# qucontrol/krotov

Hardware: AMD Instinct MI355X
Metric: state*timestep propagations/s (Krotov iterations/s in iterations_per_sec), 256-objective N=64 ensemble (higher is better)
Workload: dtype f64

## Files before the change

### include/krotov_hip.h

```cpp
#ifndef KROTOV_HIP_H
#define KROTOV_HIP_H

#include <stddef.h>
#include <stdint.h>

#ifdef __cplusplus
extern "C" {
#endif

typedef struct kh_engine kh_engine;

typedef struct kh_cdouble {
    double re, im;
} kh_cdouble;

enum kh_status {
    KH_OK = 0,
    KH_ERR_INVALID = -1,
    KH_ERR_HIP = -2,
    KH_ERR_UNSUPPORTED = -3,
    KH_ERR_TIMEOUT = -4,
    KH_ERR_NOMEM = -5
};

// ... 125 lines not shown

int kh_expect(kh_engine *engine, const kh_cdouble *states_dev, const kh_cdouble *const *e_ops, int32_t n_e,
              kh_cdouble *out_dev, void *stream);

int kh_chi_boundary(kh_engine *engine, const kh_cdouble *targets_dev,
                    const kh_cdouble *psi_T_dev, const kh_cdouble *c_dev,
                    const kh_cdouble *d_dev, kh_cdouble *chi_T_dev,
                    double *chi_norms_dev, void *stream);

int kh_check(kh_engine *engine);

int kh_last_stats(kh_engine *engine, double stats[4]);

int kh_series_tables(int32_t real_spectrum, double tol, double *theta , double *ratios );

int kh_series_tables_defect(double tol, double theta_cap, double defect, double *theta ,
                            double *ratios );

int kh_series_tables_odd(double tol, double *theta , double *c0 , double *rows );

int32_t kh_ell_rows_of(int32_t N);
int kh_ell_layout(int32_t N, int32_t n_ops, const kh_csr *ops_host, int32_t *E, int32_t *Ec, int32_t *off,
                  kh_cdouble *vals, int32_t E_cap);
int kh_ell_layout_global(int32_t N, int32_t n_ops, const kh_csr *ops_host, int32_t *E, int32_t *Ec, int32_t *off,
                         kh_cdouble *vals, int32_t E_cap);

int kh_set_row_split(kh_engine *engine, int workgroups_per_objective);
int kh_ellsplit_rows(int32_t N, int32_t S, int32_t part, int32_t *first, int32_t *count);

int kh_debug_occupy(kh_engine *engine, int32_t workgroups, double milliseconds, void *stream);

int kh_debug_launched(int32_t which, char *buf, int32_t cap);

#ifdef __cplusplus
}
#endif
#endif
```

### krotov_amd/_lib.py

```python
import ctypes
import os

_HERE = os.path.dirname(os.path.abspath(__file__))
LIB_PATH = os.path.join(_HERE, 'libkrotov_hip.so')

KH_OK = 0
KH_ERR_INVALID = -1
KH_ERR_HIP = -2
KH_ERR_UNSUPPORTED = -3
KH_ERR_TIMEOUT = -4
KH_ERR_NOMEM = -5


class kh_problem(ctypes.Structure):
    _fields_ = [
        ('K', ctypes.c_int32),
        ('N', ctypes.c_int32),
        ('L', ctypes.c_int32),
        ('nt', ctypes.c_int32),
        ('is_super', ctypes.c_int32),
        ('reserved', ctypes.c_int32),
        ('dt', ctypes.POINTER(ctypes.c_double)),
        ('ops', ctypes.POINTER(ctypes.c_void_p)),
        ('op_norms', ctypes.POINTER(ctypes.c_double)),
# ... 65 lines not shown
    'kh_backward_store_source': (ctypes.c_int, [_P] * 7),
    'kh_apply_store': (ctypes.c_int, [_P] * 6),
    'kh_forward_update': (ctypes.c_int, [_P] * 11),
    'kh_set_second_order': (ctypes.c_int, [_P, _P, _P, _P]),
    'kh_set_second_order_replicas': (ctypes.c_int, [_P, _P, _P, _P]),
    'kh_set_parametrization': (ctypes.c_int, [_P] * 7),
    'kh_update_begin': (ctypes.c_int, [_P] * 9),
    'kh_update_step': (ctypes.c_int, [_P, ctypes.c_int32] + [_P] * 9),
    'kh_update_step_dev': (ctypes.c_int, [_P] * 11),
    'kh_update_end': (ctypes.c_int, [_P, _P, _P]),
    'kh_p2p_create_window': (ctypes.c_int, [_P, ctypes.c_int32, ctypes.c_int32, _P]),
    'kh_p2p_open_peers': (ctypes.c_int, [_P, _P]),
    'kh_p2p_selftest': (ctypes.c_int, [_P, ctypes.c_int32, _P]),
    'kh_p2p_disable': (ctypes.c_int, [_P]),
    'kh_tau': (ctypes.c_int, [_P, _P, _P, _P, _P]),
    'kh_expect': (ctypes.c_int, [_P, _P, _P, ctypes.c_int32, _P, _P]),
    'kh_chi_boundary': (ctypes.c_int, [_P, _P, _P, _P, _P, _P, _P, _P]),
    'kh_check': (ctypes.c_int, [_P]),
    'kh_last_stats': (ctypes.c_int, [_P, ctypes.POINTER(ctypes.c_double)]),
    'kh_debug_occupy': (ctypes.c_int, [_P, ctypes.c_int32, ctypes.c_double, _P]),
    'kh_p2p_stats': (ctypes.c_int, [_P, ctypes.POINTER(ctypes.c_double)]),
    'kh_set_update_workgroups': (ctypes.c_int, [_P, ctypes.c_int32, ctypes.POINTER(ctypes.c_int32)]),
    'kh_set_row_split': (ctypes.c_int, [_P, ctypes.c_int]),
    'kh_ellsplit_rows': (ctypes.c_int, [ctypes.c_int32, ctypes.c_int32, ctypes.c_int32, ctypes.POINTER(ctypes.c_int32),
                                        ctypes.POINTER(ctypes.c_int32)]),
    'kh_debug_launched': (ctypes.c_int, [ctypes.c_int32, ctypes.c_char_p, ctypes.c_int32]),
    'kh_series_tables': (ctypes.c_int, [ctypes.c_int32, ctypes.c_double, ctypes.POINTER(ctypes.c_double),
                                        ctypes.POINTER(ctypes.c_double)]),
    'kh_series_tables_defect': (ctypes.c_int, [ctypes.c_double, ctypes.c_double, ctypes.c_double,
                                               ctypes.POINTER(ctypes.c_double), ctypes.POINTER(ctypes.c_double)]),
    'kh_series_tables_odd': (ctypes.c_int, [ctypes.c_double, ctypes.POINTER(ctypes.c_double),
                                            ctypes.POINTER(ctypes.c_double), ctypes.POINTER(ctypes.c_double)]),
    'kh_ell_rows_of': (ctypes.c_int32, [ctypes.c_int32]),
    'kh_ell_layout': (ctypes.c_int, [ctypes.c_int32, ctypes.c_int32, _P, ctypes.POINTER(ctypes.c_int32),
                                     ctypes.POINTER(ctypes.c_int32), _P, _P, ctypes.c_int32]),
    'kh_ell_layout_global': (ctypes.c_int, [ctypes.c_int32, ctypes.c_int32, _P, ctypes.POINTER(ctypes.c_int32),
                                            ctypes.POINTER(ctypes.c_int32), _P, _P, ctypes.c_int32]),
}

_lib = None


def load():
    global _lib
    if _lib is not None:
        return _lib
    if not os.path.exists(LIB_PATH):
        raise RuntimeError(
            "krotov_amd: %s is missing. Build it with `python __graft_entry__.py` "
            "(hipcc --offload-arch=gfx950). There is no CPU fallback." % LIB_PATH
        )
    import torch

    try:
        lib = ctypes.CDLL(LIB_PATH)
    except OSError as exc:
        raise RuntimeError("krotov_amd: cannot load %s: %s" % (LIB_PATH, exc))
    for name, (restype, argtypes) in SYMBOLS.items():
        fn = getattr(lib, name)
        fn.restype = restype
        fn.argtypes = argtypes
    _lib = lib
    return lib


def forget_launched_kernels():
# ... 24 lines not shown
```

### krotov_amd/csrc/kh_tile64.h

```cpp
#pragma once

#include "kh_common.h"
#include "kh_generic.h"

#define KH_TILE_N 64

template <bool MFMA>
struct KhLanes;
template <>
struct KhLanes<true> {
    static __device__ __forceinline__ int cg(int lane) { return (lane >> 4) + 4 * ((lane >> 2) & 1); }
    static __device__ __forceinline__ int row_in(int lane) { return (lane & 3) + 4 * ((lane >> 3) & 1); }
    static __device__ __forceinline__ int row_out(int lane) { return (lane >> 4) + 4 * ((lane >> 3) & 1); }
    static __device__ __forceinline__ double rowsum(double v, double scale) {
        const double d = __builtin_amdgcn_mfma_f64_4x4x4f64(v, scale, 0.0, 0, 0, 0);
        return d + dpp_move<KH_DPP_HALF_MIRROR>(d);
    }
    static __device__ __forceinline__ double writers_sum(double v) {
        const double d = __builtin_amdgcn_mfma_f64_4x4x4f64(v, 1.0, 0.0, 0, 0, 0);
        return d + dpp_move<KH_DPP_ROR8>(d);
    }
};
template <>
struct KhLanes<false> {
    static __device__ __forceinline__ int cg(int lane) { return lane & 7; }
    static __device__ __forceinline__ int row_in(int lane) { return lane >> 3; }
    static __device__ __forceinline__ int row_out(int lane) { return lane >> 3; }
    static __device__ __forceinline__ double rowsum(double v, double scale) { return scale * sum8(v); }
    static __device__ __forceinline__ double writers_sum(double v) { return sum64(v); }
};
typedef KhLanes<false> KhTileLanes;

template <int RPT>
struct KhTile {
    static constexpr int THREADS = 512 / RPT;
    static constexpr int WAVES = THREADS / 64;
    static __device__ __forceinline__ int row_in(int wave, int lane, int r) {
        return wave * (8 * RPT) + r * 8 + KhTileLanes::row_in(lane);
    }
    static __device__ __forceinline__ int row(int wave, int lane, int r) {
        return wave * (8 * RPT) + r * 8 + KhTileLanes::row_out(lane);
    }
    static __device__ __forceinline__ bool writer(int lane) { return (lane & 7) == 0; }
};

template <int RPT>
__device__ __forceinline__ void kh_tile_load_op(const cplx *op, int N, int wave, int lane, cplx (&a)[RPT][8]) {
    const int cg = KhTileLanes::cg(lane);
#pragma unroll
    for (int r = 0; r < RPT; ++r) {
        const int row = KhTile<RPT>::row_in(wave, lane, r);
#pragma unroll
        for (int j = 0; j < 8; ++j) {
            const int col = cg + 8 * j;
            a[r][j] = (op != nullptr && row < N && col < N) ? op[(size_t)row * N + col] : c_make(0.0, 0.0);
        }
    }
}

template <int RPT>
__device__ __forceinline__ void kh_tile_matvec(const cplx (&a)[RPT][8], const cplx *x, int cg, cplx (&y)[RPT]) {
    cplx xv[8];
#pragma unroll
    for (int j = 0; j < 8; ++j) xv[j] = x[cg + 8 * j];
#pragma unroll
// ... 158 lines not shown
```

### krotov_amd/csrc/kh_tile64q2.h

```cpp
#pragma once

#include "kh_common.h"
#include "kh_generic.h"
#include "kh_tile64.h"

#define KH_Q2_THREADS 512
#ifdef KH_Q2_DPP_REDUCE
typedef KhLanes<false> KhQ2Lanes;
#else
typedef KhLanes<true> KhQ2Lanes;
#endif
#define KH_Q2_TILE_ELEMS (8 * KH_Q2_THREADS)

struct KhQ2Lds {
    cplx *h0;
    cplx *p0;
    cplx (*buf)[KH_TILE_N];
    cplx *chib;
    cplx *sbuf;
    double *red;
    double *D;
    double2 *inv2;
    double *deg;
};

__host__ __device__ inline size_t kh_q2_lds_bytes() {
    return (size_t)2 * KH_Q2_TILE_ELEMS * sizeof(cplx) + 4 * KH_TILE_N * sizeof(cplx) + (2 * 8 * 2 + 4) * sizeof(double) +
           (KH_MAX_DEGREE / 2 + 1) * sizeof(double2) + (KH_MAX_DEGREE + 2) * sizeof(double);
}

__device__ __forceinline__ KhQ2Lds kh_q2_carve(char *smem) {
    KhQ2Lds s;
    s.h0 = (cplx *)smem;
    s.p0 = s.h0 + KH_Q2_TILE_ELEMS;
    s.buf = (cplx(*)[KH_TILE_N])(s.p0 + KH_Q2_TILE_ELEMS);
    s.chib = (cplx *)(s.buf + 2);
    s.sbuf = s.chib + KH_TILE_N;
    s.red = (double *)(s.sbuf + KH_TILE_N);
    s.D = s.red + 2 * 8 * 2;
    s.inv2 = (double2 *)(s.D + 4);
    s.deg = (double *)(s.inv2 + KH_MAX_DEGREE / 2 + 1);
    return s;
}

__device__ __forceinline__ void kh_q2_load_tile(const cplx *op, int N, int wave, int lane, cplx (&t)[8]) {
    const int row = wave * 8 + KhQ2Lanes::row_in(lane), cg = KhQ2Lanes::cg(lane);
#pragma unroll
    for (int j = 0; j < 8; ++j) {
        const int col = cg + 8 * j;
        t[j] = (op != nullptr && row < N && col < N) ? op[(size_t)row * N + col] : c_make(0.0, 0.0);
    }
}

__device__ __forceinline__ void kh_q2_stage_tile(const cplx *op, int N, int wave, int lane, int tid, cplx *dst) {
    cplx t[8];
    kh_q2_load_tile(op, N, wave, lane, t);
#pragma unroll
    for (int j = 0; j < 8; ++j) dst[j * KH_Q2_THREADS + tid] = t[j];
}

__device__ __forceinline__ void kh_q2_load_rows(const KhSweepArgs &p, const KhQ2Lds &s, int m, int tid) {
    __syncthreads();
    if (tid < KH_Q2_ROWS) {
        const double *r = p.q2_rows + ((size_t)m * KH_Q2_ROWS + tid) * 2;
        s.inv2[tid] = make_double2(r[0], r[1]);
    }
    if (tid == KH_Q2_ROWS) s.inv2[KH_Q2_ROWS] = make_double2(p.q2_c0[m], 0.0);
    __syncthreads();
}

__device__ __forceinline__ void kh_q2_build(const KhQ2Lds &s, int tid, double eps, const cplx (&h1)[8],
                                            const cplx (&p1)[8], const cplx (&p2)[8], cplx (&a)[8], cplx (&b)[8]) {
    const double eps2 = eps * eps;
#pragma unroll
    for (int j = 0; j < 8; ++j) {
        const cplx h0 = s.h0[j * KH_Q2_THREADS + tid];
        const cplx q0 = s.p0[j * KH_Q2_THREADS + tid];
        a[j].x = fma(eps, h1[j].x, h0.x);
        a[j].y = fma(eps, h1[j].y, h0.y);
        b[j].x = fma(eps2, p2[j].x, fma(eps, p1[j].x, q0.x));
        b[j].y = fma(eps2, p2[j].y, fma(eps, p1[j].y, q0.y));
    }
}

#define KH_Q2_REFRESH 64
__device__ __forceinline__ void kh_q2_restart_lds(const KhQ2Lds &s, int tid, cplx (&a)[8], cplx (&b)[8]) {
#pragma unroll
    for (int j = 0; j < 8; ++j) {
        a[j] = s.h0[j * KH_Q2_THREADS + tid];
        b[j] = s.p0[j * KH_Q2_THREADS + tid];
    }
}
__device__ __forceinline__ void kh_q2_advance_reg(double eps, double eps_prev, const cplx (&h1)[8], const cplx (&p1)[8],
                                                  const cplx (&p2)[8], cplx (&a)[8], cplx (&b)[8]) {
    const double e1 = eps - eps_prev, e2 = e1 * (eps + eps_prev);
#pragma unroll
    for (int j = 0; j < 8; ++j) {
        a[j].x = fma(e1, h1[j].x, a[j].x);
        a[j].y = fma(e1, h1[j].y, a[j].y);
        b[j].x = fma(e2, p2[j].x, fma(e1, p1[j].x, b[j].x));
        b[j].y = fma(e2, p2[j].y, fma(e1, p1[j].y, b[j].y));
    }
}

__device__ __forceinline__ void kh_q2_advance(const KhQ2Lds &s, int tid, double eps, double eps_prev, const cplx (&h1)[8],
                                              cplx (&a)[8], cplx (&b)[8]) {
    const double e1 = eps - eps_prev, e2 = e1 * (eps + eps_prev);
#pragma unroll
    for (int j = 0; j < 8; ++j) {
        const cplx q1 = s.h0[j * KH_Q2_THREADS + tid];
        const cplx q2 = s.p0[j * KH_Q2_THREADS + tid];
        a[j].x = fma(e1, h1[j].x, a[j].x);
        a[j].y = fma(e1, h1[j].y, a[j].y);
        b[j].x = fma(e2, q2.x, fma(e1, q1.x, b[j].x));
        b[j].y = fma(e2, q2.y, fma(e1, q1.y, b[j].y));
    }
}

template <class Epilogue>
__device__ __forceinline__ int kh_q2_expm_action(const cplx (&a)[8], const cplx (&b)[8], cplx &state,
                                                 cplx (*buf)[KH_TILE_N], cplx *sbuf, const double2 *inv2, int &cur,
                                                 cplx *store_in, int N, double fre, double fim,
                                                 double dt, int nsub, int m, bool odd, int wave, int lane,
                                                 Epilogue epilogue) {
    const int cg = KhQ2Lanes::cg(lane), row = wave * 8 + KhQ2Lanes::row_out(lane);
    const bool writer = (lane & 7) == 0;
    const double h = nsub == 1 ? dt : dt / nsub;
    const double f2h2 = (fre * fre - fim * fim) * h * h;
    const int phases = (m + 1) >> 1;
    const bool no_last_b = odd && (m & 1);
    if (store_in != nullptr && wave == 0 && lane < N) {
        store_in[lane] = buf[cur][lane];
    }
    for (int sub = 0; sub < nsub; ++sub) {
        const double hr = h * inv2[0].x, c0 = inv2[KH_Q2_ROWS].x;
        cplx sacc = c_make(hr * state.x, hr * state.y);
        state = c_make(c0 * state.x, c0 * state.y);
        if (phases == 1) {
            if (writer) sbuf[row] = sacc;
            __syncthreads();
        }
        for (int ph = 0; ph < phases; ++ph) {
            const bool last = (ph + 1 == phases);
            if (!(last && no_last_b)) {
                const double c2 = f2h2 * inv2[ph].y;
                cplx xv[8];
#pragma unroll
                for (int j = 0; j < 8; ++j) xv[j] = buf[cur][cg + 8 * j];
                cplx yb = c_make(0.0, 0.0);
#pragma unroll
                for (int j = 0; j < 8; ++j) c_fma(yb, b[j], xv[j]);
                const double t2x = KhQ2Lanes::rowsum(yb.x, c2), t2y = KhQ2Lanes::rowsum(yb.y, c2);
                state.x += t2x;
                state.y += t2y;
                if (!last) {
                    const double hn = h * inv2[ph + 1].x;
                    sacc.x = fma(hn, t2x, sacc.x);
                    sacc.y = fma(hn, t2y, sacc.y);
                    if (writer) {
                        buf[cur ^ 1][row] = c_make(t2x, t2y);
                        if (ph + 2 == phases) sbuf[row] = sacc;
                    }
                }
            }
            if (last) {
                __builtin_amdgcn_sched_barrier(0);
                cplx sv[8];
#pragma unroll
                for (int j = 0; j < 8; ++j) sv[j] = sbuf[cg + 8 * j];
                cplx ya = c_make(0.0, 0.0);
#pragma unroll
                for (int j = 0; j < 8; ++j) c_fma(ya, a[j], sv[j]);
                const cplx odd_sum = c_mul(c_make(fre, fim), c_make(KhQ2Lanes::rowsum(ya.x, 1.0), KhQ2Lanes::rowsum(ya.y, 1.0)));
                state.x += odd_sum.x;
                state.y += odd_sum.y;
                if (writer) buf[cur ^ 1][row] = c_make(state.x, state.y);
                if (sub + 1 == nsub) epilogue();
            }
            __syncthreads();
            cur ^= 1;
        }
    }
    return nsub * (phases + (no_last_b ? 0 : 1));
}

__global__ void __launch_bounds__(KH_Q2_THREADS)
kh_q2_sweep_store(KhSweepArgs p, const cplx *const *__restrict__ sq, const double *__restrict__ pulses,
                  const cplx *__restrict__ state_in, cplx *__restrict__ store, cplx *__restrict__ state_out,
                  int direction)
#if KH_DEFINES(KH_TU_Q2)
{
    extern __shared__ __attribute__((aligned(16))) char smem[];
    const KhQ2Lds s = kh_q2_carve(smem);
    const int tid = threadIdx.x, wave = tid >> 6, lane = tid & 63;
    if (tid <= KH_MAX_DEGREE) s.deg[tid] = p.q2_theta[tid];
    const int row = wave * 8 + KhQ2Lanes::row_out(lane);
    const bool writer = (lane & 7) == 0;
    const int N = p.N, nt = p.nt;
    double matvecs = 0.0;
    for (int k = blockIdx.x; k < p.K; k += gridDim.x) {
        const cplx *const *ops_k = p.ops + (size_t)k * 2;
        const cplx *const *sq_k = sq + (size_t)k * 3;
        __syncthreads();
        kh_q2_stage_tile(ops_k[0], N, wave, lane, tid, s.h0);
        kh_q2_stage_tile(sq_k[0], N, wave, lane, tid, s.p0);
        cplx h1[8], p1[8], p2[8];
        kh_q2_load_tile(ops_k[1], N, wave, lane, h1);
        kh_q2_load_tile(sq_k[1], N, wave, lane, p1);
        kh_q2_load_tile(sq_k[2], N, wave, lane, p2);
        const double nrm0 = p.op_norms[(size_t)k * 2], nrm1 = p.op_norms[(size_t)k * 2 + 1];

        cplx state = row < N ? state_in[(size_t)k * N + row] : c_make(0.0, 0.0);
        int cur = 0;
        if (writer) s.buf[0][row] = state;
        __syncthreads();
        const int n0 = direction > 0 ? 0 : nt - 2;
        double eps_next = pulses[n0], dt_next = p.dt[n0];
        KhDegreeCache dc = {12, 1.0, 0.0};
        int m_rows = -1;
#ifdef KH_TIMING
        long long t_build = 0, t_phases = 0;
#endif
        cplx a[8], b[8];
        double eps_prev = 0.0;
        for (int step0 = 0; step0 < nt - 1; step0 += KH_Q2_REFRESH) {
        kh_q2_restart_lds(s, tid, a, b);
        eps_prev = 0.0;
        const int step_stop = step0 + KH_Q2_REFRESH < nt - 1 ? step0 + KH_Q2_REFRESH : nt - 1;
        for (int step = step0; step < step_stop; ++step) {
#ifdef KH_TIMING
            const long long tq0 = clock64();
#endif
            const int n = direction > 0 ? step : nt - 2 - step;
            const double eps = eps_next, dt = dt_next;
            if (step + 1 < nt - 1) {
                const int nn = direction > 0 ? n + 1 : n - 1;
                dt_next = p.dt[nn];
                eps_next = pulses[nn];
            }
            int nsub, m;
            kh_degree_cached((nrm0 + fabs(eps) * nrm1) * dt, s.deg, p.theta_max, p.inv_theta_max, dc, &nsub, &m);
            if (m != m_rows) {
                kh_q2_load_rows(p, s, m, tid);
                m_rows = m;
            }
            kh_q2_advance_reg(eps, eps_prev, h1, p1, p2, a, b);
            eps_prev = eps;
            cplx *store_in =
                store == nullptr ? nullptr : store + ((size_t)k * nt + (direction > 0 ? n : n + 1)) * N;
#ifdef KH_TIMING
            const long long tq1 = clock64();
            t_build += tq1 - tq0;
#endif
            matvecs += kh_q2_expm_action(a, b, state, s.buf, s.sbuf, s.inv2, cur, store_in, N, p.fre, p.fim, dt, nsub, m,
                                         p.q2_odd != 0, wave, lane, [] {});
#ifdef KH_TIMING
            t_phases += clock64() - tq1;
#endif
        }
        }
#ifdef KH_TIMING
        if (tid == 0 && k == 0 && p.stats != nullptr) {
            p.stats[1] = (double)t_build;
            p.stats[2] = (double)t_phases;
        }
#endif
        if (store != nullptr && wave == 0 && lane < N)
            store[((size_t)k * nt + (direction > 0 ? nt - 1 : 0)) * N + lane] = s.buf[cur][lane];
        if (state_out != nullptr && wave == 0 && lane < N) state_out[(size_t)k * N + lane] = s.buf[cur][lane];
    }
    if (tid == 0 && p.stats != nullptr) atomicAdd(p.stats, matvecs);
}
#else
    ;
#endif

template <bool SO, bool ADJ, bool SINGLE = false>
__global__ void __launch_bounds__(KH_Q2_THREADS)
kh_q2_forward_update(KhSweepArgs p, const cplx *const *__restrict__ sq, KhUpdateArgs u, KhExchange ex) {
    static_assert(!(SO && ADJ), "the second-order bra depends on the new state");
#ifdef KH_Q2_NO_PREFETCH
    constexpr bool PREFETCH = false;
#else
    constexpr bool PREFETCH = !SO;
#endif
#ifdef KH_Q2_NARROW_POLL
    constexpr bool WIDE_POLL = false;
#else
    constexpr bool WIDE_POLL = true;
#endif
    if (u.n_dev != nullptr) {
        u.n_begin = *u.n_dev;
        u.n_end = u.n_begin + 1;
        if (u.n_begin >= p.nt - 1) return;
    }
    extern __shared__ __attribute__((aligned(16))) char smem[];
    const KhQ2Lds s = kh_q2_carve(smem);
    double(*red)[8][2] = (double(*)[8][2])s.red;
    double(*D_sh)[2] = (double(*)[2])s.D;
    const int tid = threadIdx.x, wave = tid >> 6, lane = tid & 63, cg = KhQ2Lanes::cg(lane);
    if (tid <= KH_MAX_DEGREE) s.deg[tid] = p.q2_theta[tid];
    const int row = wave * 8 + KhQ2Lanes::row_out(lane);
    if (wave < 4) __builtin_amdgcn_s_setprio(1);
    const bool writer = (lane & 7) == 0;
    const int N = p.N, nt = p.nt;
    const int k = blockIdx.x;
    double matvecs = 0.0;

    const cplx *const *ops_k = p.ops + (size_t)k * 2;
    const cplx *const *sq_k = sq + (size_t)k * 3;
    kh_q2_stage_tile(sq_k[1], N, wave, lane, tid, s.h0);
    kh_q2_stage_tile(sq_k[2], N, wave, lane, tid, s.p0);
    cplx h1[8], a[8], b[8];
    kh_q2_load_tile(ops_k[1], N, wave, lane, h1);
    double eps_prev = 0.0;
    const double nrm0 = kh_uniform(p.op_norms[(size_t)k * 2]), nrm1 = kh_uniform(p.op_norms[(size_t)k * 2 + 1]);
    const double chi_norm = kh_uniform(u.chi_norms[k]);

    cplx state = row < N ? u.phi[(size_t)k * N + row] : c_make(0.0, 0.0);
    int cur = 0;
    if (writer) s.buf[0][row] = state;
    __syncthreads();

    double g_a_loc = 0.0;
    cplx chi = c_make(0.0, 0.0), prev = c_make(0.0, 0.0);
    double hs = 0.0;
    auto load_chi = [&](int n) {
        chi = row < N ? u.chi_store[((size_t)k * nt + n) * N + row] : c_make(0.0, 0.0);
        if constexpr (SO) {
            prev = row < N ? u.fw_prev[((size_t)k * nt + n) * N + row] : c_make(0.0, 0.0);
            hs = 0.5 * u.sigma[n] / chi_norm;
        }
    };

    auto partial_pieces = [&](int par) {
        cplx xv[8];
#pragma unroll
        for (int j = 0; j < 8; ++j) xv[j] = s.buf[cur][cg + 8 * j];
        cplx y = c_make(0.0, 0.0);
#pragma unroll
        for (int j = 0; j < 8; ++j) c_fma(y, h1[j], xv[j]);
        y.x = KhQ2Lanes::rowsum(y.x, 1.0);
        y.y = KhQ2Lanes::rowsum(y.y, 1.0);
        cplx ov = c_make(0.0, 0.0);
        cplx bra = chi;
        if constexpr (SO) bra = c_make(fma(hs, state.x - prev.x, chi.x), fma(hs, state.y - prev.y, chi.y));
        if (writer) c_fma_conj(ov, bra, y);
        const double v = KhQ2Lanes::writers_sum(u.mu_re * ov.y + u.mu_im * ov.x);
        if (lane == 0) red[par][wave][0] = v;
        matvecs += 1.0;
    };
    auto partial_total = [&](int par) {
        double acc = 0.0;
#pragma unroll
        for (int w = 0; w < 8; ++w) acc += red[par][w][0];
        return chi_norm * acc;
    };

    cplx w = c_make(0.0, 0.0);
    auto adjoint_side = [&]() {
        cplx xv[8];
#pragma unroll
        for (int j = 0; j < 8; ++j) xv[j] = s.chib[cg + 8 * j];
        cplx y = c_make(0.0, 0.0);
#pragma unroll
        for (int j = 0; j < 8; ++j) c_fma(y, h1[j], xv[j]);
        w.x = KhQ2Lanes::rowsum(y.x, u.adj_sign);
        w.y = KhQ2Lanes::rowsum(y.y, u.adj_sign);
        matvecs += 1.0;
    };

    if (u.n_begin < nt - 1) {
        load_chi(u.n_begin);
        partial_pieces(u.n_begin & 1);
    }
    if constexpr (ADJ) {
        if (u.n_begin + 1 < nt - 1) {
            load_chi(u.n_begin + 1);
            if (writer) s.chib[row] = chi;
        }
    }
    __syncthreads();

    double dt_next = kh_uniform(p.dt[u.n_begin]), guess_next = kh_uniform(u.guess[u.n_begin]),
           shape_next = kh_uniform(u.shape[u.n_begin]);
    const double lam = kh_uniform(u.lambda[0]);
    int m_rows = -1;
    double stepw_next = kh_uniform(shape_next / lam);
    KhDegreeCache dc = {12, 1.0, 0.0};

#ifdef KH_TIMING
    long long t_ex = 0, t_prop = 0, t_part = 0, t_coll = 0;
    const long long t_all0 = clock64();
#endif
    for (int nr = u.n_begin, n_stop; nr < u.n_end; nr = n_stop) {
    kh_q2_load_tile(ops_k[0], N, wave, lane, a);
    kh_q2_load_tile(sq_k[0], N, wave, lane, b);
    eps_prev = 0.0;
    n_stop = (nr / KH_Q2_REFRESH + 1) * KH_Q2_REFRESH;
    n_stop = n_stop < u.n_end ? n_stop : u.n_end;
    for (int n = nr; n < n_stop; ++n) {
        const int par = n & 1;
        if constexpr (!ADJ) {
            if (n + 1 < nt - 1) load_chi(n + 1);
        }
#ifdef KH_TIMING
        const long long tq0 = clock64();
#endif
        cplx q1[8], q2[8];
        {
            double part[1] = {0.0};
            if (wave == 0) {
                part[0] = partial_total(par);
#ifndef KH_Q2_X_NOEXCH
                kh_exchange_publish(ex, n, k, 1, lane, part);
#endif
            }
            if constexpr (PREFETCH) {
#pragma unroll
                for (int j = 0; j < 8; ++j) {
                    q1[j] = s.h0[j * KH_Q2_THREADS + tid];
                    q2[j] = s.p0[j * KH_Q2_THREADS + tid];
                }
            }
            if constexpr (ADJ) {
                if (n + 1 < nt - 1) adjoint_side();
            }
            if (wave == 0) {
                double D[1];
#ifdef KH_Q2_X_NOEXCH
// ... 33 lines not shown
        dt_next = kh_uniform(dt_ld);
        guess_next = kh_uniform(guess_ld);
        shape_next = kh_uniform(shape_ld);
        if (k == 0 && tid == 0) u.opt[n] = eps;
        int nsub, m;
        kh_degree_cached((nrm0 + fabs(eps) * nrm1) * dt, s.deg, p.theta_max, p.inv_theta_max, dc, &nsub, &m);
        if (m != m_rows) {
            kh_q2_load_rows(p, s, m, tid);
            m_rows = m;
        }
        if constexpr (PREFETCH)
            kh_q2_advance_reg(eps, eps_prev, h1, q1, q2, a, b);
        else
            kh_q2_advance(s, tid, eps, eps_prev, h1, a, b);
        eps_prev = eps;
        stepw_next = kh_uniform(shape_next / lam);
        cplx *fw_out = nullptr;
        if constexpr (SO) fw_out = u.fw_store + ((size_t)k * nt + n) * N;
        if constexpr (ADJ) {
            if (n + 2 < nt - 1) load_chi(n + 2);
            auto epilogue = [&] {
                if (n + 1 < nt - 1) {
                    cplx ov = c_make(0.0, 0.0);
                    if (writer) c_fma_conj(ov, w, state);
                    const double v = KhQ2Lanes::writers_sum(u.mu_re * ov.y + u.mu_im * ov.x);
                    if (lane == 0) red[(n + 1) & 1][wave][0] = v;
                    if (n + 2 < nt - 1 && writer) s.chib[row] = chi;
                }
            };
#ifdef KH_Q2_X_NOPHASES
            epilogue();
            __syncthreads();
#else
            matvecs += kh_q2_expm_action(a, b, state, s.buf, s.sbuf, s.inv2, cur, fw_out, N, p.fre, p.fim, dt, nsub, m,
                                         p.q2_odd != 0, wave, lane, epilogue);
#endif
        } else {
            matvecs += kh_q2_expm_action(a, b, state, s.buf, s.sbuf, s.inv2, cur, fw_out, N, p.fre, p.fim, dt, nsub, m,
                                         p.q2_odd != 0, wave, lane, [] {});
        }
#ifdef KH_TIMING
        const long long tq2 = clock64();
        t_prop += tq2 - tq1;
#endif
        if constexpr (!ADJ) {
            if (n + 1 < nt - 1) {
                partial_pieces((n + 1) & 1);
                __syncthreads();
            }
        }
#ifdef KH_TIMING
        t_part += clock64() - tq2;
#endif
    }
    }
#ifdef KH_TIMING
    if (tid == 0 && k == 0 && p.stats != nullptr) {
        p.stats[1] = (double)t_ex;
        p.stats[2] = (double)t_prop;
        p.stats[3] = (double)t_coll;
    }
#endif
    if (wave == 0 && lane < N) {
        u.phi[(size_t)k * N + lane] = s.buf[cur][lane];
        if constexpr (SO) u.fw_store[((size_t)k * nt + u.n_end) * N + lane] = s.buf[cur][lane];
    }
    if (k == 0 && tid == 0) u.g_a[0] = g_a_loc;
    if (tid == 0 && p.stats != nullptr) atomicAdd(p.stats, matvecs);
}

__global__ void kh_q2_product(const cplx *__restrict__ X, const cplx *__restrict__ Y, cplx *__restrict__ C, int N,
                              int symmetrize)
#if KH_DEFINES(KH_TU_MAIN)
{
    for (int idx = blockIdx.x * blockDim.x + threadIdx.x; idx < N * N; idx += gridDim.x * blockDim.x) {
        const int i = idx / N, j = idx % N;
        cplx acc = c_make(0.0, 0.0);
        for (int q = 0; q < N; ++q) c_fma(acc, X[(size_t)i * N + q], Y[(size_t)q * N + j]);
        if (symmetrize)
            for (int q = 0; q < N; ++q) c_fma(acc, Y[(size_t)i * N + q], X[(size_t)q * N + j]);
        C[idx] = acc;
    }
}
#else
    ;
#endif
```

### krotov_amd/csrc/krotov_hip.hip

```cpp
#include <hip/hip_runtime.h>

#include <cxxabi.h>
#include <dlfcn.h>

#include <cmath>
#include <cstdarg>
#include <cstdio>
#include <cstdlib>
#include <algorithm>
#include <atomic>
#include <climits>
#include <cstring>
#include <deque>
#include <map>
#include <mutex>
#include <set>
#include <string>
#include <tuple>
#include <type_traits>
#include <utility>
#include <vector>

#include "../../include/krotov_hip.h"
#include "kh_common.h"
// ... 2979 lines not shown

extern "C" int kh_last_stats(kh_engine *e, double stats[4]) {
    if (e == nullptr || stats == nullptr) return kh_fail(KH_ERR_INVALID, "null argument");
    double d[4] = {0, 0, 0, 0};
    KH_HIP(hipMemcpy(d, e->d_stats, sizeof(d), hipMemcpyDeviceToHost));
    stats[0] = d[0];
    stats[1] = e->last_intervals;
    stats[2] = e->last_wgs;
    stats[3] = 0.0;
#ifdef KH_TIMING
    stats[0] = d[0];
    stats[1] = d[1];
    stats[2] = d[2];
    stats[3] = d[3];
    if (getenv("KH_TRACE")) {
        double tr[64];
        KH_HIP(hipMemcpy(tr, e->d_stats + 4, sizeof(tr), hipMemcpyDeviceToHost));
        fprintf(stderr, "KH_TRACE (cycles since the interval's start):");
        for (int i = 0; i < 64 && (i == 0 || tr[i] != 0.0); ++i) fprintf(stderr, " %d:%.0f", i, tr[i] - tr[0]);
        fprintf(stderr, "\n");
        unsigned int ab[2] = {0, 0};
        KH_HIP(hipMemcpy(ab, e->d_abort, sizeof(ab), hipMemcpyDeviceToHost));
        fprintf(stderr, "KH_TRACE polling rounds of workgroup 0 since the engine was created: %u\n", ab[1]);
        fprintf(stderr, "KH_TRACE raw [16..31]:");
        for (int i = 16; i < 32; ++i) fprintf(stderr, " %.0f", tr[i]);
        fprintf(stderr, "\n");
    }
#endif
    return KH_OK;
}

extern "C" int32_t kh_ell_rows_of(int32_t N) { return N >= 1 && N <= KH_ELL_NMAX ? kh_ell_rows(N) : 0; }

static int ell_layout(int32_t N, int32_t n_ops, const kh_csr *ops_host, int32_t *E_out, int32_t *Ec_out, int32_t *off_out,
                      kh_cdouble *vals_out, int32_t E_cap, bool global) {
    if (ops_host == nullptr || E_out == nullptr || Ec_out == nullptr || n_ops < 1 || N < 1)
        return kh_fail(KH_ERR_INVALID, "bad argument");
    const int nmax = global ? KH_ELLG_NMAX : KH_ELL_NMAX;
    if (N > nmax) return kh_fail(KH_ERR_UNSUPPORTED, "N = %d: the padded row form serves N <= %d", N, nmax);
    std::vector<HostCsr> host(n_ops);
    std::vector<const HostCsr *> ptrs(n_ops, nullptr);
    for (int o = 0; o < n_ops; ++o) {
        if (ops_host[o].data == nullptr) continue;
        if (!canonical_csr(ops_host[o].indptr, ops_host[o].indices, (const cplx *)ops_host[o].data, ops_host[o].nnz, N, host[o]))
            return kh_fail(KH_ERR_INVALID, "operator %d: inconsistent CSR arrays", o);
        ptrs[o] = &host[o];
    }
    std::vector<int> off;
    std::vector<cplx> vals;
    int E = 0, Ec = 0;
    if (!build_ell_host(ptrs, N, off, vals, E, Ec, global, global))
        return kh_fail(KH_ERR_UNSUPPORTED, "rows wider than the kernels' register budget (%d entries for N = %d)", kh_ell_emax(N), N);
    *E_out = E;
    *Ec_out = Ec;
    if (off_out != nullptr || vals_out != nullptr) {
        if (E_cap < E) return kh_fail(KH_ERR_INVALID, "E_cap = %d < E = %d", E_cap, E);
        if (off_out != nullptr) memcpy(off_out, off.data(), sizeof(int) * off.size());
        if (vals_out != nullptr) memcpy(vals_out, vals.data(), sizeof(cplx) * vals.size());
    }
    return KH_OK;
}

extern "C" int kh_ell_layout(int32_t N, int32_t n_ops, const kh_csr *ops_host, int32_t *E_out, int32_t *Ec_out, int32_t *off_out,
                             kh_cdouble *vals_out, int32_t E_cap) {
    return ell_layout(N, n_ops, ops_host, E_out, Ec_out, off_out, vals_out, E_cap, false);
}
// ... 6 lines not shown
```

Baseline: 69.16 million.

## Use 16-row lane map with DPP broadcast dot in backward q2 sweep

Adds an alternative lane-to-matrix mapping for the q2 sweep kernel. Each wave handles 16 rows, and the row dot product broadcasts one x element per lane across the DPP row with v_fmac_f64_dpp, using an MFMA 4x4 row sum. The vector buffers are split into two halves that are summed on read. This replaces the 8 LDS reads per lane in each matvec with a single read plus register broadcasts. The new mapping is used only for the backward direction by default, and it adds inline assembly, extra LDS space and a two-half buffer layout that the other kernels must index as [0].

```diff
diff --git a/include/krotov_hip.h b/include/krotov_hip.h
--- a/include/krotov_hip.h
+++ b/include/krotov_hip.h
@@ -181,6 +181,8 @@
 
 int kh_debug_launched(int32_t which, char *buf, int32_t cap);
 
+int kh_debug_q2_lane_map(int32_t wave, int32_t lane, int32_t *out );
+
 #ifdef __cplusplus
 }
 #endif
diff --git a/krotov_amd/_lib.py b/krotov_amd/_lib.py
--- a/krotov_amd/_lib.py
+++ b/krotov_amd/_lib.py
@@ -121,6 +121,7 @@
     'kh_series_tables_odd': (ctypes.c_int, [ctypes.c_double, ctypes.POINTER(ctypes.c_double),
                                             ctypes.POINTER(ctypes.c_double), ctypes.POINTER(ctypes.c_double)]),
     'kh_ell_rows_of': (ctypes.c_int32, [ctypes.c_int32]),
+    'kh_debug_q2_lane_map': (ctypes.c_int, [ctypes.c_int32, ctypes.c_int32, ctypes.POINTER(ctypes.c_int32)]),
     'kh_ell_layout': (ctypes.c_int, [ctypes.c_int32, ctypes.c_int32, _P, ctypes.POINTER(ctypes.c_int32),
                                      ctypes.POINTER(ctypes.c_int32), _P, _P, ctypes.c_int32]),
     'kh_ell_layout_global': (ctypes.c_int, [ctypes.c_int32, ctypes.c_int32, _P, ctypes.POINTER(ctypes.c_int32),
diff --git a/krotov_amd/csrc/kh_tile64.h b/krotov_amd/csrc/kh_tile64.h
--- a/krotov_amd/csrc/kh_tile64.h
+++ b/krotov_amd/csrc/kh_tile64.h
@@ -31,6 +31,37 @@
 };
 typedef KhLanes<false> KhTileLanes;
 
+struct KhLanesR16 {
+    static __host__ __device__ __forceinline__ int half(int wave) { return wave & 1; }
+    static __host__ __device__ __forceinline__ int row_in(int wave, int lane) { return 16 * (wave >> 1) + (lane & 15); }
+    static __host__ __device__ __forceinline__ int col0(int wave, int lane) { return 8 * ((lane >> 4) + 4 * (wave & 1)); }
+    static __host__ __device__ __forceinline__ int x_index(int wave, int lane) { return col0(wave, lane) + (lane & 7); }
+    static __host__ __device__ __forceinline__ int landing_lane(int lane) { return 16 * (lane & 3) + 4 * ((lane >> 2) & 3); }
+    static __host__ __device__ __forceinline__ int row_out(int wave, int lane) {
+        return 16 * (wave >> 1) + 4 * ((lane >> 2) & 3) + (lane >> 4);
+    }
+    static __host__ __device__ __forceinline__ bool writer(int lane) { return (lane & 3) == 0; }
+    static __device__ __forceinline__ double rowsum(double v, double scale) {
+        return __builtin_amdgcn_mfma_f64_4x4x4f64(v, scale, 0.0, 0, 0, 0);
+    }
+#define KH_R16_FMAC(J, RE, IM)                                                           \
+    "v_fmac_f64_dpp %0, %2, %" #RE " row_newbcast:" #J " row_mask:0xf bank_mask:0xf\n\t"  \
+    "v_fmac_f64_dpp %1, %3, %" #RE " row_newbcast:" #J " row_mask:0xf bank_mask:0xf\n\t"  \
+    "v_fmac_f64_dpp %0, -%3, %" #IM " row_newbcast:" #J " row_mask:0xf bank_mask:0xf\n\t" \
+    "v_fmac_f64_dpp %1, %2, %" #IM " row_newbcast:" #J " row_mask:0xf bank_mask:0xf\n\t"
+    static __device__ __forceinline__ void dot8(cplx &acc, const cplx (&t)[8], cplx x) {
+        asm("s_nop 1\n\t"
+            KH_R16_FMAC(0, 4, 5) KH_R16_FMAC(1, 6, 7) KH_R16_FMAC(2, 8, 9) KH_R16_FMAC(3, 10, 11)
+            KH_R16_FMAC(4, 12, 13) KH_R16_FMAC(5, 14, 15) KH_R16_FMAC(6, 16, 17) KH_R16_FMAC(7, 18, 19)
+            "s_nop 1"
+            : "+v"(acc.x), "+v"(acc.y)
+            : "v"(x.x), "v"(x.y), "v"(t[0].x), "v"(t[0].y), "v"(t[1].x), "v"(t[1].y), "v"(t[2].x), "v"(t[2].y),
+              "v"(t[3].x), "v"(t[3].y), "v"(t[4].x), "v"(t[4].y), "v"(t[5].x), "v"(t[5].y), "v"(t[6].x), "v"(t[6].y),
+              "v"(t[7].x), "v"(t[7].y));
+    }
+#undef KH_R16_FMAC
+};
+
 template <int RPT>
 struct KhTile {
     static constexpr int THREADS = 512 / RPT;
diff --git a/krotov_amd/csrc/kh_tile64q2.h b/krotov_amd/csrc/kh_tile64q2.h
--- a/krotov_amd/csrc/kh_tile64q2.h
+++ b/krotov_amd/csrc/kh_tile64q2.h
@@ -12,12 +12,39 @@
 #endif
 #define KH_Q2_TILE_ELEMS (8 * KH_Q2_THREADS)
 
+#ifdef KH_Q2_LDS_BROADCAST
+constexpr bool KH_Q2_R16 = false;
+#else
+constexpr bool KH_Q2_R16 = true;
+#endif
+
+template <bool R16>
+struct KhQ2Map;
+template <>
+struct KhQ2Map<false> {
+    static __device__ __forceinline__ int half(int) { return 0; }
+    static __device__ __forceinline__ int row_in(int wave, int lane) { return wave * 8 + KhQ2Lanes::row_in(lane); }
+    static __device__ __forceinline__ int col(int, int lane, int j) { return KhQ2Lanes::cg(lane) + 8 * j; }
+    static __device__ __forceinline__ int row_out(int wave, int lane) { return wave * 8 + KhQ2Lanes::row_out(lane); }
+    static __device__ __forceinline__ bool writer(int lane) { return (lane & 7) == 0; }
+    static __device__ __forceinline__ double rowsum(double v, double scale) { return KhQ2Lanes::rowsum(v, scale); }
+};
+template <>
+struct KhQ2Map<true> {
+    static __device__ __forceinline__ int half(int wave) { return KhLanesR16::half(wave); }
+    static __device__ __forceinline__ int row_in(int wave, int lane) { return KhLanesR16::row_in(wave, lane); }
+    static __device__ __forceinline__ int col(int wave, int lane, int j) { return KhLanesR16::col0(wave, lane) + j; }
+    static __device__ __forceinline__ int row_out(int wave, int lane) { return KhLanesR16::row_out(wave, lane); }
+    static __device__ __forceinline__ bool writer(int lane) { return KhLanesR16::writer(lane); }
+    static __device__ __forceinline__ double rowsum(double v, double scale) { return KhLanesR16::rowsum(v, scale); }
+};
+
 struct KhQ2Lds {
     cplx *h0;
     cplx *p0;
-    cplx (*buf)[KH_TILE_N];
+    cplx (*buf)[2][KH_TILE_N];
     cplx *chib;
-    cplx *sbuf;
+    cplx (*sbuf)[KH_TILE_N];
     double *red;
     double *D;
     double2 *inv2;
@@ -25,7 +52,7 @@
 };
 
 __host__ __device__ inline size_t kh_q2_lds_bytes() {
-    return (size_t)2 * KH_Q2_TILE_ELEMS * sizeof(cplx) + 4 * KH_TILE_N * sizeof(cplx) + (2 * 8 * 2 + 4) * sizeof(double) +
+    return (size_t)2 * KH_Q2_TILE_ELEMS * sizeof(cplx) + 7 * KH_TILE_N * sizeof(cplx) + (2 * 8 * 2 + 4) * sizeof(double) +
            (KH_MAX_DEGREE / 2 + 1) * sizeof(double2) + (KH_MAX_DEGREE + 2) * sizeof(double);
 }
 
@@ -33,28 +60,30 @@
     KhQ2Lds s;
     s.h0 = (cplx *)smem;
     s.p0 = s.h0 + KH_Q2_TILE_ELEMS;
-    s.buf = (cplx(*)[KH_TILE_N])(s.p0 + KH_Q2_TILE_ELEMS);
+    s.buf = (cplx(*)[2][KH_TILE_N])(s.p0 + KH_Q2_TILE_ELEMS);
     s.chib = (cplx *)(s.buf + 2);
-    s.sbuf = s.chib + KH_TILE_N;
-    s.red = (double *)(s.sbuf + KH_TILE_N);
+    s.sbuf = (cplx(*)[KH_TILE_N])(s.chib + KH_TILE_N);
+    s.red = (double *)(s.sbuf + 2);
     s.D = s.red + 2 * 8 * 2;
     s.inv2 = (double2 *)(s.D + 4);
     s.deg = (double *)(s.inv2 + KH_MAX_DEGREE / 2 + 1);
     return s;
 }
 
+template <bool R16>
 __device__ __forceinline__ void kh_q2_load_tile(const cplx *op, int N, int wave, int lane, cplx (&t)[8]) {
-    const int row = wave * 8 + KhQ2Lanes::row_in(lane), cg = KhQ2Lanes::cg(lane);
+    const int row = KhQ2Map<R16>::row_in(wave, lane);
 #pragma unroll
     for (int j = 0; j < 8; ++j) {
-        const int col = cg + 8 * j;
+        const int col = KhQ2Map<R16>::col(wave, lane, j);
         t[j] = (op != nullptr && row < N && col < N) ? op[(size_t)row * N + col] : c_make(0.0, 0.0);
     }
 }
 
+template <bool R16>
 __device__ __forceinline__ void kh_q2_stage_tile(const cplx *op, int N, int wave, int lane, int tid, cplx *dst) {
     cplx t[8];
-    kh_q2_load_tile(op, N, wave, lane, t);
+    kh_q2_load_tile<R16>(op, N, wave, lane, t);
 #pragma unroll
     for (int j = 0; j < 8; ++j) dst[j * KH_Q2_THREADS + tid] = t[j];
 }
@@ -67,6 +96,33 @@
     }
     if (tid == KH_Q2_ROWS) s.inv2[KH_Q2_ROWS] = make_double2(p.q2_c0[m], 0.0);
     __syncthreads();
+}
+
+template <bool R16>
+__device__ __forceinline__ cplx kh_q2_dot(const cplx (&t)[8], const cplx *x0, const cplx *x1, int wave, int lane) {
+    cplx acc = c_make(0.0, 0.0);
+    if constexpr (R16) {
+        const int xi = KhLanesR16::x_index(wave, lane);
+        const cplx xa = x0[xi], xb = x1[xi];
+        KhLanesR16::dot8(acc, t, c_make(xa.x + xb.x, xa.y + xb.y));
+    } else {
+        const int cg = KhQ2Lanes::cg(lane);
+        cplx xv[8];
+#pragma unroll
+        for (int j = 0; j < 8; ++j) xv[j] = x0[cg + 8 * j];
+#pragma unroll
+        for (int j = 0; j < 8; ++j) c_fma(acc, t[j], xv[j]);
+    }
+    return acc;
+}
+template <bool R16>
+__device__ __forceinline__ cplx kh_q2_vec_at(const cplx (*v)[KH_TILE_N], int i) {
+    cplx x = v[0][i];
+    if constexpr (R16) {
+        x.x += v[1][i].x;
+        x.y += v[1][i].y;
+    }
+    return x;
 }
 
 __device__ __forceinline__ void kh_q2_build(const KhQ2Lds &s, int tid, double eps, const cplx (&h1)[8],
@@ -117,64 +173,67 @@
     }
 }
 
-template <class Epilogue>
+template <bool R16, class Epilogue>
 __device__ __forceinline__ int kh_q2_expm_action(const cplx (&a)[8], const cplx (&b)[8], cplx &state,
-                                                 cplx (*buf)[KH_TILE_N], cplx *sbuf, const double2 *inv2, int &cur,
-                                                 cplx *store_in, int N, double fre, double fim,
+                                                 cplx (*buf)[2][KH_TILE_N], cplx (*sbuf)[KH_TILE_N], const double2 *inv2,
+                                                 int &cur, cplx *store_in, int N, double fre, double fim,
                                                  double dt, int nsub, int m, bool odd, int wave, int lane,
                                                  Epilogue epilogue) {
-    const int cg = KhQ2Lanes::cg(lane), row = wave * 8 + KhQ2Lanes::row_out(lane);
-    const bool writer = (lane & 7) == 0;
+    typedef KhQ2Map<R16> Map;
+    const int row = Map::row_out(wave, lane), half = Map::half(wave);
+    const bool writer = Map::writer(lane);
     const double h = nsub == 1 ? dt : dt / nsub;
     const double f2h2 = (fre * fre - fim * fim) * h * h;
     const int phases = (m + 1) >> 1;
     const bool no_last_b = odd && (m & 1);
     if (store_in != nullptr && wave == 0 && lane < N) {
-        store_in[lane] = buf[cur][lane];
+        store_in[lane] = kh_q2_vec_at<R16>(buf[cur], lane);
     }
     for (int sub = 0; sub < nsub; ++sub) {
         const double hr = h * inv2[0].x, c0 = inv2[KH_Q2_ROWS].x;
         cplx sacc = c_make(hr * state.x, hr * state.y);
         state = c_make(c0 * state.x, c0 * state.y);
         if (phases == 1) {
-            if (writer) sbuf[row] = sacc;
+            if (writer) sbuf[half][row] = sacc;
             __syncthreads();
         }
         for (int ph = 0; ph < phases; ++ph) {
             const bool last = (ph + 1 == phases);
             if (!(last && no_last_b)) {
-                const double c2 = f2h2 * inv2[ph].y;
-                cplx xv[8];
-#pragma unroll
-                for (int j = 0; j < 8; ++j) xv[j] = buf[cur][cg + 8 * j];
-                cplx yb = c_make(0.0, 0.0);
-#pragma unroll
-                for (int j = 0; j < 8; ++j) c_fma(yb, b[j], xv[j]);
-                const double t2x = KhQ2Lanes::rowsum(yb.x, c2), t2y = KhQ2Lanes::rowsum(yb.y, c2);
+                double c2, hn = 0.0;
+                cplx yb;
+                if constexpr (R16) {
+                    const int xi = KhLanesR16::x_index(wave, lane);
+                    const cplx x0 = buf[cur][0][xi], x1 = buf[cur][1][xi];
+                    const double r2 = inv2[ph].y, r1n = inv2[ph + 1].x;
+                    c2 = f2h2 * r2;
+                    hn = h * r1n;
+                    yb = c_make(0.0, 0.0);
+                    KhLanesR16::dot8(yb, b, c_make(x0.x + x1.x, x0.y + x1.y));
+                } else {
+                    c2 = f2h2 * inv2[ph].y;
+                    yb = kh_q2_dot<R16>(b, buf[cur][0], buf[cur][1], wave, lane);
+                }
+                const double t2x = Map::rowsum(yb.x, c2), t2y = Map::rowsum(yb.y, c2);
                 state.x += t2x;
                 state.y += t2y;
                 if (!last) {
-                    const double hn = h * inv2[ph + 1].x;
+                    if constexpr (!R16) hn = h * inv2[ph + 1].x;
                     sacc.x = fma(hn, t2x, sacc.x);
                     sacc.y = fma(hn, t2y, sacc.y);
                     if (writer) {
-                        buf[cur ^ 1][row] = c_make(t2x, t2y);
-                        if (ph + 2 == phases) sbuf[row] = sacc;
+                        buf[cur ^ 1][half][row] = c_make(t2x, t2y);
+                        if (ph + 2 == phases) sbuf[half][row] = sacc;
                     }
                 }
             }
             if (last) {
                 __builtin_amdgcn_sched_barrier(0);
-                cplx sv[8];
-#pragma unroll
-                for (int j = 0; j < 8; ++j) sv[j] = sbuf[cg + 8 * j];
-                cplx ya = c_make(0.0, 0.0);
-#pragma unroll
-                for (int j = 0; j < 8; ++j) c_fma(ya, a[j], sv[j]);
-                const cplx odd_sum = c_mul(c_make(fre, fim), c_make(KhQ2Lanes::rowsum(ya.x, 1.0), KhQ2Lanes::rowsum(ya.y, 1.0)));
+                const cplx ya = kh_q2_dot<R16>(a, sbuf[0], sbuf[1], wave, lane);
+                const cplx odd_sum = c_mul(c_make(fre, fim), c_make(Map::rowsum(ya.x, 1.0), Map::rowsum(ya.y, 1.0)));
                 state.x += odd_sum.x;
                 state.y += odd_sum.y;
-                if (writer) buf[cur ^ 1][row] = c_make(state.x, state.y);
+                if (writer) buf[cur ^ 1][half][row] = c_make(state.x, state.y);
                 if (sub + 1 == nsub) epilogue();
             }
             __syncthreads();
@@ -182,6 +241,95 @@
         }
     }
     return nsub * (phases + (no_last_b ? 0 : 1));
+}
+
+template <bool R16>
+__device__ __forceinline__ void kh_q2_sweep_store_body(const KhSweepArgs &p, const cplx *const *__restrict__ sq,
+                                                       const double *__restrict__ pulses,
+                                                       const cplx *__restrict__ state_in, cplx *__restrict__ store,
+                                                       cplx *__restrict__ state_out, int direction, char *smem) {
+    const KhQ2Lds s = kh_q2_carve(smem);
+    const int tid = threadIdx.x, wave = tid >> 6, lane = tid & 63;
+    if (tid <= KH_MAX_DEGREE) s.deg[tid] = p.q2_theta[tid];
+    typedef KhQ2Map<R16> Map;
+    const int row = Map::row_out(wave, lane);
+    const int half = Map::half(wave);
+    const bool writer = Map::writer(lane);
+    const int N = p.N, nt = p.nt;
+    double matvecs = 0.0;
+    for (int k = blockIdx.x; k < p.K; k += gridDim.x) {
+        const cplx *const *ops_k = p.ops + (size_t)k * 2;
+        const cplx *const *sq_k = sq + (size_t)k * 3;
+        __syncthreads();
+        kh_q2_stage_tile<R16>(ops_k[0], N, wave, lane, tid, s.h0);
+        kh_q2_stage_tile<R16>(sq_k[0], N, wave, lane, tid, s.p0);
+        cplx h1[8], p1[8], p2[8];
+        kh_q2_load_tile<R16>(ops_k[1], N, wave, lane, h1);
+        kh_q2_load_tile<R16>(sq_k[1], N, wave, lane, p1);
+        kh_q2_load_tile<R16>(sq_k[2], N, wave, lane, p2);
+        const double nrm0 = p.op_norms[(size_t)k * 2], nrm1 = p.op_norms[(size_t)k * 2 + 1];
+
+        cplx state = (row < N && half == 0) ? state_in[(size_t)k * N + row] : c_make(0.0, 0.0);
+        int cur = 0;
+        if (writer) s.buf[0][half][row] = state;
+        __syncthreads();
+        const int n0 = direction > 0 ? 0 : nt - 2;
+        double eps_next = pulses[n0], dt_next = p.dt[n0];
+        KhDegreeCache dc = {12, 1.0, 0.0};
+        int m_rows = -1;
+#ifdef KH_TIMING
+        long long t_build = 0, t_phases = 0;
+#endif
+        cplx a[8], b[8];
+        double eps_prev = 0.0;
+        for (int step0 = 0; step0 < nt - 1; step0 += KH_Q2_REFRESH) {
+        kh_q2_restart_lds(s, tid, a, b);
+        eps_prev = 0.0;
+        const int step_stop = step0 + KH_Q2_REFRESH < nt - 1 ? step0 + KH_Q2_REFRESH : nt - 1;
+        for (int step = step0; step < step_stop; ++step) {
+#ifdef KH_TIMING
+            const long long tq0 = clock64();
+#endif
+            const int n = direction > 0 ? step : nt - 2 - step;
+            const double eps = eps_next, dt = dt_next;
+            if (step + 1 < nt - 1) {
+                const int nn = direction > 0 ? n + 1 : n - 1;
+                dt_next = p.dt[nn];
+                eps_next = pulses[nn];
+            }
+            int nsub, m;
+            kh_degree_cached((nrm0 + fabs(eps) * nrm1) * dt, s.deg, p.theta_max, p.inv_theta_max, dc, &nsub, &m);
+            if (m != m_rows) {
+                kh_q2_load_rows(p, s, m, tid);
+                m_rows = m;
+            }
+            kh_q2_advance_reg(eps, eps_prev, h1, p1, p2, a, b);
+            eps_prev = eps;
+            cplx *store_in =
+                store == nullptr ? nullptr : store + ((size_t)k * nt + (direction > 0 ? n : n + 1)) * N;
+#ifdef KH_TIMING
+            const long long tq1 = clock64();
+            t_build += tq1 - tq0;
+#endif
+            matvecs += kh_q2_expm_action<R16>(a, b, state, s.buf, s.sbuf, s.inv2, cur, store_in, N, p.fre, p.fim, dt, nsub,
+                                              m, p.q2_odd != 0, wave, lane, [] {});
+#ifdef KH_TIMING
+            t_phases += clock64() - tq1;
+#endif
+        }
+        }
+#ifdef KH_TIMING
+        if (tid == 0 && k == 0 && p.stats != nullptr) {
+            p.stats[1] = (double)t_build;
+            p.stats[2] = (double)t_phases;
+        }
+#endif
+        if (store != nullptr && wave == 0 && lane < N)
+            store[((size_t)k * nt + (direction > 0 ? nt - 1 : 0)) * N + lane] = kh_q2_vec_at<R16>(s.buf[cur], lane);
+        if (state_out != nullptr && wave == 0 && lane < N)
+            state_out[(size_t)k * N + lane] = kh_q2_vec_at<R16>(s.buf[cur], lane);
+    }
+    if (tid == 0 && p.stats != nullptr) atomicAdd(p.stats, matvecs);
 }
 
 __global__ void __launch_bounds__(KH_Q2_THREADS)
@@ -191,85 +339,10 @@
 #if KH_DEFINES(KH_TU_Q2)
 {
     extern __shared__ __attribute__((aligned(16))) char smem[];
-    const KhQ2Lds s = kh_q2_carve(smem);
-    const int tid = threadIdx.x, wave = tid >> 6, lane = tid & 63;
-    if (tid <= KH_MAX_DEGREE) s.deg[tid] = p.q2_theta[tid];
-    const int row = wave * 8 + KhQ2Lanes::row_out(lane);
-    const bool writer = (lane & 7) == 0;
-    const int N = p.N, nt = p.nt;
-    double matvecs = 0.0;
-    for (int k = blockIdx.x; k < p.K; k += gridDim.x) {
-        const cplx *const *ops_k = p.ops + (size_t)k * 2;
-        const cplx *const *sq_k = sq + (size_t)k * 3;
-        __syncthreads();
-        kh_q2_stage_tile(ops_k[0], N, wave, lane, tid, s.h0);
-        kh_q2_stage_tile(sq_k[0], N, wave, lane, tid, s.p0);
-        cplx h1[8], p1[8], p2[8];
-        kh_q2_load_tile(ops_k[1], N, wave, lane, h1);
-        kh_q2_load_tile(sq_k[1], N, wave, lane, p1);
-        kh_q2_load_tile(sq_k[2], N, wave, lane, p2);
-        const double nrm0 = p.op_norms[(size_t)k * 2], nrm1 = p.op_norms[(size_t)k * 2 + 1];
-
-        cplx state = row < N ? state_in[(size_t)k * N + row] : c_make(0.0, 0.0);
-        int cur = 0;
-        if (writer) s.buf[0][row] = state;
-        __syncthreads();
-        const int n0 = direction > 0 ? 0 : nt - 2;
-        double eps_next = pulses[n0], dt_next = p.dt[n0];
-        KhDegreeCache dc = {12, 1.0, 0.0};
-        int m_rows = -1;
-#ifdef KH_TIMING
-        long long t_build = 0, t_phases = 0;
-#endif
-        cplx a[8], b[8];
-        double eps_prev = 0.0;
-        for (int step0 = 0; step0 < nt - 1; step0 += KH_Q2_REFRESH) {
-        kh_q2_restart_lds(s, tid, a, b);
-        eps_prev = 0.0;
-        const int step_stop = step0 + KH_Q2_REFRESH < nt - 1 ? step0 + KH_Q2_REFRESH : nt - 1;
-        for (int step = step0; step < step_stop; ++step) {
-#ifdef KH_TIMING
-            const long long tq0 = clock64();
-#endif
-            const int n = direction > 0 ? step : nt - 2 - step;
-            const double eps = eps_next, dt = dt_next;
-            if (step + 1 < nt - 1) {
-                const int nn = direction > 0 ? n + 1 : n - 1;
-                dt_next = p.dt[nn];
-                eps_next = pulses[nn];
-            }
-            int nsub, m;
-            kh_degree_cached((nrm0 + fabs(eps) * nrm1) * dt, s.deg, p.theta_max, p.inv_theta_max, dc, &nsub, &m);
-            if (m != m_rows) {
-                kh_q2_load_rows(p, s, m, tid);
-                m_rows = m;
-            }
-            kh_q2_advance_reg(eps, eps_prev, h1, p1, p2, a, b);
-            eps_prev = eps;
-            cplx *store_in =
-                store == nullptr ? nullptr : store + ((size_t)k * nt + (direction > 0 ? n : n + 1)) * N;
-#ifdef KH_TIMING
-            const long long tq1 = clock64();
-            t_build += tq1 - tq0;
-#endif
-            matvecs += kh_q2_expm_action(a, b, state, s.buf, s.sbuf, s.inv2, cur, store_in, N, p.fre, p.fim, dt, nsub, m,
-                                         p.q2_odd != 0, wave, lane, [] {});
-#ifdef KH_TIMING
-            t_phases += clock64() - tq1;
-#endif
-        }
-        }
-#ifdef KH_TIMING
-        if (tid == 0 && k == 0 && p.stats != nullptr) {
-            p.stats[1] = (double)t_build;
-            p.stats[2] = (double)t_phases;
-        }
-#endif
-        if (store != nullptr && wave == 0 && lane < N)
-            store[((size_t)k * nt + (direction > 0 ? nt - 1 : 0)) * N + lane] = s.buf[cur][lane];
-        if (state_out != nullptr && wave == 0 && lane < N) state_out[(size_t)k * N + lane] = s.buf[cur][lane];
-    }
-    if (tid == 0 && p.stats != nullptr) atomicAdd(p.stats, matvecs);
+    if (KH_Q2_R16 && !(direction > 0))
+        kh_q2_sweep_store_body<true>(p, sq, pulses, state_in, store, state_out, direction, smem);
+    else
+        kh_q2_sweep_store_body<false>(p, sq, pulses, state_in, store, state_out, direction, smem);
 }
 #else
     ;
@@ -309,17 +382,17 @@
 
     const cplx *const *ops_k = p.ops + (size_t)k * 2;
     const cplx *const *sq_k = sq + (size_t)k * 3;
-    kh_q2_stage_tile(sq_k[1], N, wave, lane, tid, s.h0);
-    kh_q2_stage_tile(sq_k[2], N, wave, lane, tid, s.p0);
+    kh_q2_stage_tile<false>(sq_k[1], N, wave, lane, tid, s.h0);
+    kh_q2_stage_tile<false>(sq_k[2], N, wave, lane, tid, s.p0);
     cplx h1[8], a[8], b[8];
-    kh_q2_load_tile(ops_k[1], N, wave, lane, h1);
+    kh_q2_load_tile<false>(ops_k[1], N, wave, lane, h1);
     double eps_prev = 0.0;
     const double nrm0 = kh_uniform(p.op_norms[(size_t)k * 2]), nrm1 = kh_uniform(p.op_norms[(size_t)k * 2 + 1]);
     const double chi_norm = kh_uniform(u.chi_norms[k]);
 
     cplx state = row < N ? u.phi[(size_t)k * N + row] : c_make(0.0, 0.0);
     int cur = 0;
-    if (writer) s.buf[0][row] = state;
+    if (writer) s.buf[0][0][row] = state;
     __syncthreads();
 
     double g_a_loc = 0.0;
@@ -336,7 +409,7 @@
     auto partial_pieces = [&](int par) {
         cplx xv[8];
 #pragma unroll
-        for (int j = 0; j < 8; ++j) xv[j] = s.buf[cur][cg + 8 * j];
+        for (int j = 0; j < 8; ++j) xv[j] = s.buf[cur][0][cg + 8 * j];
         cplx y = c_make(0.0, 0.0);
 #pragma unroll
         for (int j = 0; j < 8; ++j) c_fma(y, h1[j], xv[j]);
@@ -394,8 +467,8 @@
     const long long t_all0 = clock64();
 #endif
     for (int nr = u.n_begin, n_stop; nr < u.n_end; nr = n_stop) {
-    kh_q2_load_tile(ops_k[0], N, wave, lane, a);
-    kh_q2_load_tile(sq_k[0], N, wave, lane, b);
+    kh_q2_load_tile<false>(ops_k[0], N, wave, lane, a);
+    kh_q2_load_tile<false>(sq_k[0], N, wave, lane, b);
     eps_prev = 0.0;
     n_stop = (nr / KH_Q2_REFRESH + 1) * KH_Q2_REFRESH;
     n_stop = n_stop < u.n_end ? n_stop : u.n_end;
@@ -495,11 +568,11 @@
             epilogue();
             __syncthreads();
 #else
-            matvecs += kh_q2_expm_action(a, b, state, s.buf, s.sbuf, s.inv2, cur, fw_out, N, p.fre, p.fim, dt, nsub, m,
+            matvecs += kh_q2_expm_action<false>(a, b, state, s.buf, s.sbuf, s.inv2, cur, fw_out, N, p.fre, p.fim, dt, nsub, m,
                                          p.q2_odd != 0, wave, lane, epilogue);
 #endif
         } else {
-            matvecs += kh_q2_expm_action(a, b, state, s.buf, s.sbuf, s.inv2, cur, fw_out, N, p.fre, p.fim, dt, nsub, m,
+            matvecs += kh_q2_expm_action<false>(a, b, state, s.buf, s.sbuf, s.inv2, cur, fw_out, N, p.fre, p.fim, dt, nsub, m,
                                          p.q2_odd != 0, wave, lane, [] {});
         }
 #ifdef KH_TIMING
@@ -525,8 +598,8 @@
     }
 #endif
     if (wave == 0 && lane < N) {
-        u.phi[(size_t)k * N + lane] = s.buf[cur][lane];
-        if constexpr (SO) u.fw_store[((size_t)k * nt + u.n_end) * N + lane] = s.buf[cur][lane];
+        u.phi[(size_t)k * N + lane] = s.buf[cur][0][lane];
+        if constexpr (SO) u.fw_store[((size_t)k * nt + u.n_end) * N + lane] = s.buf[cur][0][lane];
     }
     if (k == 0 && tid == 0) u.g_a[0] = g_a_loc;
     if (tid == 0 && p.stats != nullptr) atomicAdd(p.stats, matvecs);
diff --git a/krotov_amd/csrc/krotov_hip.hip b/krotov_amd/csrc/krotov_hip.hip
--- a/krotov_amd/csrc/krotov_hip.hip
+++ b/krotov_amd/csrc/krotov_hip.hip
@@ -3035,6 +3035,19 @@
 
 extern "C" int32_t kh_ell_rows_of(int32_t N) { return N >= 1 && N <= KH_ELL_NMAX ? kh_ell_rows(N) : 0; }
 
+extern "C" int kh_debug_q2_lane_map(int32_t wave, int32_t lane, int32_t *out) {
+    if (out == nullptr || wave < 0 || wave >= KH_Q2_THREADS / 64 || lane < 0 || lane >= 64)
+        return kh_fail(KH_ERR_INVALID, "bad argument");
+    out[0] = KhLanesR16::row_in(wave, lane);
+    out[1] = KhLanesR16::col0(wave, lane);
+    out[2] = KhLanesR16::x_index(wave, lane);
+    out[3] = KhLanesR16::landing_lane(lane);
+    out[4] = KhLanesR16::row_out(wave, lane);
+    out[5] = KhLanesR16::writer(lane) ? 1 : 0;
+    out[6] = KhLanesR16::half(wave);
+    return KH_OK;
+}
+
 static int ell_layout(int32_t N, int32_t n_ops, const kh_csr *ops_host, int32_t *E_out, int32_t *Ec_out, int32_t *off_out,
                       kh_cdouble *vals_out, int32_t E_cap, bool global) {
     if (ops_host == nullptr || E_out == nullptr || Ec_out == nullptr || n_ops < 1 || N < 1)
```

After: 71.08 million, median of 6. 1.03x the previous value.
